# imperatormk/candle-birefnet

Hardware: AMD Instinct MI355X
Metric: images/sec @1024x1024 Swin-L (higher is better)
Workload: dtype f32 storage+accumulate; GEMM operands as two fp16 planes of the power-of-two-scaled operand (22-bit mantissa), 3 fp16 MFMAs/product (fp32-equivalent inside the fp16 range: |GEMM input| < 8190); 1 GPU; BASELINE configs[1]: Swin-L 1024x1024 batch=1 fp32 on 1xMI355X (single-image latency); batch_per_gpu=1, global_batch=1, size=1024, deform_mode=reference_cpu, compute=f32_half2, streams_per_gpu=1, branch_streams_per_gpu=5, inputs=resident in HBM (torch cuda tensors), weights: synthetic seed 42

## Files before the change

candle_birefnet_amd/csrc/kernels/window_attention.hip:

```cpp
#include "../brn_kernels.h"
#include "split_planes.h"
#include <cstdlib>
#include <type_traits>

namespace brn {

typedef float f32x4 __attribute__((ext_vector_type(4)));

constexpr int WS = 12;
constexpr int NTOK = 144;
constexpr int HD = 32;
constexpr int KV_LD = 36;
constexpr int ATT_THREADS = 192;

template <int IOB>
__device__ __forceinline__ f32x4 att_load4(const float* base, long off) {
    if constexpr (IOB != 0) {
        using E = std::conditional_t<IOB == 2, _Float16, __bf16>;
        typedef E ex4_ld __attribute__((ext_vector_type(4)));
        const ex4_ld h = *reinterpret_cast<const ex4_ld*>(reinterpret_cast<const E*>(base) + off);
        return f32x4{(float)h[0], (float)h[1], (float)h[2], (float)h[3]};
    } else return *reinterpret_cast<const f32x4*>(base + off);
}
template <int IOB>
__device__ __forceinline__ f32x4 att_bias4(const float* bias) {
    f32x4 v = *reinterpret_cast<const f32x4*>(bias);
    if constexpr (IOB != 0) {
        using E = std::conditional_t<IOB == 2, _Float16, __bf16>;
#pragma unroll
        for (int e = 0; e < 4; ++e) v[e] = (float)(E)v[e];
    }
    return v;
}
template <int WSZ, int NWV = 3, int IOB = 0>
__global__ void __launch_bounds__(NWV * 64) window_attention_f32_kernel(const WindowAttnParams pa, const WindowAttnParams pb, const int nblk0) {
    constexpr int WS = WSZ, NTOK = WSZ * WSZ, NT16 = (NTOK + 15) / 16, NPADTOK = NT16 * 16;
    constexpr int NTHR = NWV * 64;
    const bool second = (int)blockIdx.x >= nblk0;
    const WindowAttnParams& p = second ? pb : pa;
    __shared__ __attribute__((aligned(16))) float Ks[NPADTOK * KV_LD];
    __shared__ __attribute__((aligned(16))) float Vs[NPADTOK * KV_LD];
    __shared__ int src_s[NPADTOK];
    __shared__ int rid_s[NPADTOK];
    __shared__ float tab_s[(2 * WS - 1) * (2 * WS - 1)];

    const int tid = threadIdx.x, lane = tid & 63, wave = tid >> 6;
    const int head = blockIdx.y;
    const int nWw = p.Wp / WS, nW = (p.Hp / WS) * nWw;
    const int bw = second ? (int)blockIdx.x - nblk0 : (int)blockIdx.x;
    const int b = bw / nW, w = bw - b * nW;
    const int wr = w / nWw, wc = w - wr * nWw;
    const int C = p.C, C3 = 3 * C;

    if (tid < NTOK) {
        const int ti = tid / WS, tj = tid - ti * WS;
        const int ph = wr * WS + ti, pw = wc * WS + tj;
        int sh = ph + p.shift, sw = pw + p.shift;
        if (sh >= p.Hp) sh -= p.Hp;
        if (sw >= p.Wp) sw -= p.Wp;
        src_s[tid] = (sh < p.H && sw < p.W) ? (b * p.H + sh) * p.W + sw : -1;
        const int fh = ph < p.Hp - WS ? 0 : (ph < p.Hp - p.shift ? 1 : 2);
        const int fw = pw < p.Wp - WS ? 0 : (pw < p.Wp - p.shift ? 1 : 2);
        rid_s[tid] = fh * 3 + fw;
    } else if (tid < NPADTOK) { src_s[tid] = -1; rid_s[tid] = 0; }
    constexpr int TABN = (2 * WS - 1) * (2 * WS - 1);
    constexpr bool REV = WS == 12;
    constexpr float LOG2E = 1.4426950408889634f;
    for (int i = tid; i < TABN; i += NTHR) tab_s[i] = REV ? LOG2E * p.rel_table[head * TABN + (TABN - 1 - i)] : p.rel_table[head * TABN + i];
    const bool has_mask = p.shift > 0 && (wr == p.Hp / WS - 1 || wc == nWw - 1);
    __syncthreads();

    for (int idx = tid; idx < NPADTOK * 8; idx += NTHR) {
        const int t = idx >> 3, c4 = (idx & 7) * 4;
        const int src = src_s[t];
        f32x4 kv, vv;
        if (src >= 0) { kv = att_load4<IOB>(p.qkv, (long)src * C3 + C + head * HD + c4); vv = att_load4<IOB>(p.qkv, (long)src * C3 + 2 * C + head * HD + c4); }
        else { kv = att_bias4<IOB>(p.qkv_bias + C + head * HD + c4); vv = att_bias4<IOB>(p.qkv_bias + 2 * C + head * HD + c4); }
        if (t >= NTOK) { kv = f32x4{0.f, 0.f, 0.f, 0.f}; vv = kv; }
        *reinterpret_cast<f32x4*>(Ks + t * KV_LD + c4) = kv;
        *reinterpret_cast<f32x4*>(Vs + t * KV_LD + c4) = vv;
    }
    __syncthreads();

    const int li = lane & 15, g = lane >> 4;

    auto load_q = [&](int qt, f32x4& q0, f32x4& q1) {
        const int qs = src_s[qt * 16 + li];
        if (qs >= 0) { q0 = att_load4<IOB>(p.qkv, (long)qs * C3 + head * HD + g * 8); q1 = att_load4<IOB>(p.qkv, (long)qs * C3 + head * HD + g * 8 + 4); }
        else { q0 = att_bias4<IOB>(p.qkv_bias + head * HD + g * 8); q1 = att_bias4<IOB>(p.qkv_bias + head * HD + g * 8 + 4); }
    };
    f32x4 qn0 = {0.f, 0.f, 0.f, 0.f}, qn1 = qn0;
    if (wave < NT16) load_q(wave, qn0, qn1);
    for (int qt = wave; qt < NT16; qt += NWV) {
        const int qtok = qt * 16 + li;
        const int qsrc = src_s[qtok];
        const int qrid = rid_s[qtok];
        const int qt_ = qtok < NTOK ? qtok : NTOK - 1;
        const int qbase = (qt_ / WS + WS - 1) * (2 * WS - 1) + (qt_ % WS) + WS - 1;
        float qf[8];
#pragma unroll
        for (int e = 0; e < 4; ++e) { qf[e] = qn0[e] * p.scale; qf[4 + e] = qn1[e] * p.scale; }
        if (qt + NWV < NT16) load_q(qt + NWV, qn0, qn1);
        f32x4 st[NT16];
#pragma unroll
        for (int kt = 0; kt < NT16; ++kt) {
            const float* kp = Ks + (kt * 16 + li) * KV_LD + g * 8;
            const f32x4 k0 = *reinterpret_cast<const f32x4*>(kp);
            const f32x4 k1 = *reinterpret_cast<const f32x4*>(kp + 4);
            f32x4 acc = {0.f, 0.f, 0.f, 0.f};
#pragma unroll
            for (int e = 0; e < 4; ++e) acc = __builtin_amdgcn_mfma_f32_16x16x4f32(k0[e], qf[e], acc, 0, 0, 0);
#pragma unroll
            for (int e = 0; e < 4; ++e) acc = __builtin_amdgcn_mfma_f32_16x16x4f32(k1[e], qf[4 + e], acc, 0, 0, 0);
            st[kt] = acc;
            if (kt % 3 == 2) __builtin_amdgcn_sched_barrier(0);
        }
        float mx = -3.0e38f;
        if constexpr (REV) {
            const int qrev = (TABN - 1) - qbase;
#pragma unroll
            for (int kt = 0; kt < NT16; ++kt) {
                const int key0 = kt * 16 + g * 4;
                const float* tb = tab_s + qrev + key0 + (WS - 1) * (key0 / WS);
#pragma unroll
                for (int r = 0; r < 4; ++r) st[kt][r] = fmaf(st[kt][r], LOG2E, tb[r]);
            }
            if (has_mask) {
#pragma unroll
                for (int kt = 0; kt < NT16; ++kt) {
#pragma unroll
                    for (int r = 0; r < 4; ++r) st[kt][r] += (rid_s[kt * 16 + g * 4 + r] != qrid) ? -100.0f * LOG2E : 0.0f;
                }
            }
#pragma unroll
            for (int kt = 0; kt < NT16; ++kt) mx = fmaxf(fmaxf(mx, fmaxf(st[kt][0], st[kt][1])), fmaxf(st[kt][2], st[kt][3]));
        } else {
#pragma unroll
            for (int kt = 0; kt < NT16; ++kt) {
#pragma unroll
                for (int r = 0; r < 4; ++r) {
                    const int key = kt * 16 + g * 4 + r;
                    const int kk = key < NTOK ? key : 0;
                    float s = st[kt][r] + tab_s[max(0, qbase - kk - (WS - 1) * (kk / WS))];
                    if (p.shift > 0) s += (rid_s[key] != qrid) ? -100.0f : 0.0f;
                    if (NTOK % 16 != 0 && key >= NTOK) s = -3.0e38f;
                    st[kt][r] = s;
                    mx = fmaxf(mx, s);
                }
            }
        }
        mx = fmaxf(mx, __shfl_xor(mx, 16));
        mx = fmaxf(mx, __shfl_xor(mx, 32));
        float sum = 0.f;
#pragma unroll
        for (int kt = 0; kt < NT16; ++kt) {
#pragma unroll
            for (int r = 0; r < 4; ++r) {
                const float e = REV ? __builtin_amdgcn_exp2f(st[kt][r] - mx) : __expf(st[kt][r] - mx);
                st[kt][r] = e;
                sum += e;
            }
        }
        sum += __shfl_xor(sum, 16);
        sum += __shfl_xor(sum, 32);
        f32x4 o0 = {0.f, 0.f, 0.f, 0.f}, o1 = {0.f, 0.f, 0.f, 0.f};
#pragma unroll
        for (int kt = 0; kt < NT16; ++kt) {
#pragma unroll
            for (int r = 0; r < 4; ++r) {
                const float* vp = Vs + (kt * 16 + g * 4 + r) * KV_LD + li;
                o0 = __builtin_amdgcn_mfma_f32_16x16x4f32(vp[0], st[kt][r], o0, 0, 0, 0);
                o1 = __builtin_amdgcn_mfma_f32_16x16x4f32(vp[16], st[kt][r], o1, 0, 0, 0);
            }
            if (kt % 2 == 1) __builtin_amdgcn_sched_barrier(0);
        }
        if (qsrc >= 0 && qtok < NTOK) {
            const float inv = 1.0f / sum;
            if (p.out_planes == 3) {
                float* orow = p.out + (long)qsrc * (C + C / 2);
                store_planes<3>(orow, head * HD + g * 4, o0 * inv);
                store_planes<3>(orow, head * HD + 16 + g * 4, o1 * inv);
            } else if (p.out_planes == 2) {
                float* orow = p.out + (long)qsrc * C;
                store_planes_h(orow, head * HD + g * 4, o0 * inv, p.out_h2);
                store_planes_h(orow, head * HD + 16 + g * 4, o1 * inv, p.out_h2);
            } else if constexpr (IOB != 0) {
                using E = std::conditional_t<IOB == 2, _Float16, __bf16>;
                typedef E ex4_st __attribute__((ext_vector_type(4)));
                E* op = reinterpret_cast<E*>(p.out) + (long)qsrc * C + head * HD + g * 4;
                ex4_st h0, h1;
#pragma unroll
                for (int e = 0; e < 4; ++e) { h0[e] = (E)(o0[e] * inv); h1[e] = (E)(o1[e] * inv); }
                *reinterpret_cast<ex4_st*>(op) = h0;
                *reinterpret_cast<ex4_st*>(op + 16) = h1;
            } else {
                float* op = p.out + (long)qsrc * C + head * HD + g * 4;
                *reinterpret_cast<f32x4*>(op) = o0 * inv;
                *reinterpret_cast<f32x4*>(op + 16) = o1 * inv;
            }
        }
    }
}

typedef __bf16 bf16x8 __attribute__((ext_vector_type(8)));
typedef __bf16 bf16x4 __attribute__((ext_vector_type(4)));
typedef __bf16 bf16x2 __attribute__((ext_vector_type(2)));
constexpr int VT_LD = 148;

__device__ __forceinline__ int kswz(int key) { return (0x78 >> (2 * ((key >> 2) & 3))) & 3; }

constexpr float ATT_H_QKV = 8.0f, ATT_H_P = 2048.0f;
template <int NP, bool H = false>
__global__ void __launch_bounds__(ATT_THREADS) window_attention_split_kernel(const WindowAttnParams pa, const WindowAttnParams pb, const int nblk0) {
    static_assert(!H || NP == 2, "fp16 planes come in pairs");
    const bool second = (int)blockIdx.x >= nblk0;
    const WindowAttnParams& p = second ? pb : pa;
    __shared__ __attribute__((aligned(16))) __bf16 Kp[NP * NTOK * HD];
    __shared__ __attribute__((aligned(16))) __bf16 Vt[NP * HD * VT_LD];
    __shared__ float tab_s[(2 * WS - 1) * (2 * WS - 1)];
    __shared__ int src_s[NTOK];
    __shared__ unsigned char rid_s[NTOK];

    const int tid = threadIdx.x, lane = tid & 63, wave = tid >> 6;
    const int head = blockIdx.y;
    const int nWw = p.Wp / WS, nW = (p.Hp / WS) * nWw;
    const int bw = second ? (int)blockIdx.x - nblk0 : (int)blockIdx.x;
    const int b = bw / nW, w = bw - b * nW;
    const int wr = w / nWw, wc = w - wr * nWw;
    const int C = p.C, C3 = 3 * C;

    if (tid < NTOK) {
        const int ti = tid / WS, tj = tid - ti * WS;
        const int ph = wr * WS + ti, pw = wc * WS + tj;
        int sh = ph + p.shift, sw = pw + p.shift;
        if (sh >= p.Hp) sh -= p.Hp;
        if (sw >= p.Wp) sw -= p.Wp;
        src_s[tid] = (sh < p.H && sw < p.W) ? (b * p.H + sh) * p.W + sw : -1;
        const int fh = ph < p.Hp - WS ? 0 : (ph < p.Hp - p.shift ? 1 : 2);
        const int fw = pw < p.Wp - WS ? 0 : (pw < p.Wp - p.shift ? 1 : 2);
        rid_s[tid] = (unsigned char)(fh * 3 + fw);
    }
    for (int i = tid; i < (2 * WS - 1) * (2 * WS - 1); i += ATT_THREADS) tab_s[i] = p.rel_table[head * ((2 * WS - 1) * (2 * WS - 1)) + i];
    __syncthreads();

    for (int idx = tid; idx < (NTOK / 2) * 8; idx += ATT_THREADS) {
        const int tp = idx >> 3, c4 = (idx & 7) * 4;
        f32x4 kv[2], vv[2];
#pragma unroll
        for (int u = 0; u < 2; ++u) {
            const int t = tp * 2 + u, src = src_s[t];
            const float* kp = src >= 0 ? p.qkv + (long)src * C3 + C + head * HD + c4 : p.qkv_bias + C + head * HD + c4;
            kv[u] = *reinterpret_cast<const f32x4*>(kp);
            vv[u] = *reinterpret_cast<const f32x4*>(kp + C);
        }
        if constexpr (H) {
#pragma unroll
            for (int u = 0; u < 2; ++u) {
                const int t = tp * 2 + u;
                bf16x4 sp[2];
                split4h<false>(kv[u], 0xffffffffu, ATT_H_QKV, sp);
#pragma unroll
                for (int pl = 0; pl < 2; ++pl)
                    *reinterpret_cast<bf16x4*>(Kp + (pl * NTOK + t) * HD + (((c4 >> 3) ^ kswz(t)) << 3) + (c4 & 4)) = sp[pl];
            }
#pragma unroll
            for (int e = 0; e < 4; ++e) {
                unsigned hi, lo;
                split_pair_h(vv[0][e], vv[1][e], ATT_H_QKV, hi, lo);
                *reinterpret_cast<unsigned*>(Vt + (c4 + e) * VT_LD + tp * 2) = hi;
                *reinterpret_cast<unsigned*>(Vt + (HD + c4 + e) * VT_LD + tp * 2) = lo;
            }
        } else {
#pragma unroll
        for (int u = 0; u < 2; ++u) {
            const int t = tp * 2 + u;
            f32x4 r = kv[u];
#pragma unroll
            for (int pl = 0; pl < NP; ++pl) {
                bf16x4 h;
#pragma unroll
                for (int e = 0; e < 4; ++e) h[e] = (__bf16)r[e];
                *reinterpret_cast<bf16x4*>(Kp + (pl * NTOK + t) * HD + (((c4 >> 3) ^ kswz(t)) << 3) + (c4 & 4)) = h;
                if (pl + 1 < NP) {
#pragma unroll
                    for (int e = 0; e < 4; ++e) r[e] -= (float)h[e];
                }
            }
        }
        f32x4 r0 = vv[0], r1 = vv[1];
#pragma unroll
        for (int pl = 0; pl < NP; ++pl) {
#pragma unroll
            for (int e = 0; e < 4; ++e) {
                bf16x2 h;
                h[0] = (__bf16)r0[e]; h[1] = (__bf16)r1[e];
                *reinterpret_cast<bf16x2*>(Vt + (pl * HD + c4 + e) * VT_LD + tp * 2) = h;
                if (pl + 1 < NP) { r0[e] -= (float)h[0]; r1[e] -= (float)h[1]; }
            }
        }
        }
    }
    __syncthreads();

    const int li = lane & 15, g = lane >> 4;
    for (int qt = wave; qt < 9; qt += 3) {
        const int qtok = qt * 16 + li;
        const int qsrc = src_s[qtok];
        const int qrid = rid_s[qtok];
        const int qbase = (qtok / WS + WS - 1) * (2 * WS - 1) + (qtok % WS) + WS - 1;
        bf16x8 qf[NP];
        {
            const float* qp = qsrc >= 0 ? p.qkv + (long)qsrc * C3 + head * HD + g * 8 : p.qkv_bias + head * HD + g * 8;
            const f32x4 q0 = *reinterpret_cast<const f32x4*>(qp);
            const f32x4 q1 = *reinterpret_cast<const f32x4*>(qp + 4);
            float r[8];
#pragma unroll
            for (int e = 0; e < 4; ++e) { r[e] = q0[e] * p.scale; r[4 + e] = q1[e] * p.scale; }
            if constexpr (H) {
                typedef unsigned u32x4_q __attribute__((ext_vector_type(4)));
                u32x4_q hi, lo;
#pragma unroll
                for (int e = 0; e < 4; ++e) { unsigned a, b2; split_pair_h(r[2 * e], r[2 * e + 1], ATT_H_QKV, a, b2); hi[e] = a; lo[e] = b2; }
                qf[0] = __builtin_bit_cast(bf16x8, hi);
                qf[1] = __builtin_bit_cast(bf16x8, lo);
            } else {
#pragma unroll
            for (int pl = 0; pl < NP; ++pl) {
#pragma unroll
                for (int e = 0; e < 8; ++e) {
                    const __bf16 h = (__bf16)r[e];
                    qf[pl][e] = h;
                    r[e] -= (float)h;
                }
            }
            }
        }
        f32x4 st[9];
#pragma unroll
        for (int kt = 0; kt < 9; ++kt) {
            const int key = kt * 16 + li;
            bf16x8 kf[NP];
#pragma unroll
            for (int pl = 0; pl < NP; ++pl)
                kf[pl] = *reinterpret_cast<const bf16x8*>(Kp + (pl * NTOK + key) * HD + ((g ^ kswz(key)) << 3));
            f32x4 acc = {0.f, 0.f, 0.f, 0.f};
            if constexpr (H) {
                acc = __builtin_amdgcn_mfma_f32_16x16x32_f16(__builtin_bit_cast(f16x8, kf[1]), __builtin_bit_cast(f16x8, qf[0]), acc, 0, 0, 0);
                acc = __builtin_amdgcn_mfma_f32_16x16x32_f16(__builtin_bit_cast(f16x8, kf[0]), __builtin_bit_cast(f16x8, qf[1]), acc, 0, 0, 0);
                acc = __builtin_amdgcn_mfma_f32_16x16x32_f16(__builtin_bit_cast(f16x8, kf[0]), __builtin_bit_cast(f16x8, qf[0]), acc, 0, 0, 0);
            } else {
            if (NP == 2) {
                acc = __builtin_amdgcn_mfma_f32_16x16x32_bf16(kf[1], qf[0], acc, 0, 0, 0);
                acc = __builtin_amdgcn_mfma_f32_16x16x32_bf16(kf[0], qf[1], acc, 0, 0, 0);
            }
            acc = __builtin_amdgcn_mfma_f32_16x16x32_bf16(kf[0], qf[0], acc, 0, 0, 0);
            }
            st[kt] = acc;
            if (kt % 3 == 2) __builtin_amdgcn_sched_barrier(0);
        }
        float mx = -3.0e38f;
#pragma unroll
        for (int kt = 0; kt < 9; ++kt) {
#pragma unroll
            for (int r = 0; r < 4; ++r) {
                const int key = kt * 16 + g * 4 + r;
                float sv = H ? fmaf(st[kt][r], 1.0f / (ATT_H_QKV * ATT_H_QKV), tab_s[qbase - key - 11 * (key / WS)]) : st[kt][r] + tab_s[qbase - key - 11 * (key / WS)];
                if (p.shift > 0) sv += ((int)rid_s[key] != qrid) ? -100.0f : 0.0f;
                st[kt][r] = sv;
                mx = fmaxf(mx, sv);
            }
        }
        mx = fmaxf(mx, __shfl_xor(mx, 16));
        mx = fmaxf(mx, __shfl_xor(mx, 32));
        float sum = 0.f;
#pragma unroll
        for (int kt = 0; kt < 9; ++kt) {
#pragma unroll
            for (int r = 0; r < 4; ++r) {
                const float e = __expf(st[kt][r] - mx);
                st[kt][r] = e;
                sum += e;
            }
        }
        sum += __shfl_xor(sum, 16);
        sum += __shfl_xor(sum, 32);
        f32x4 o0 = {0.f, 0.f, 0.f, 0.f}, o1 = {0.f, 0.f, 0.f, 0.f};
#pragma unroll
        for (int t = 0; t < 5; ++t) {
            bf16x8 pf[NP];
            {
                float r[8];
#pragma unroll
                for (int e = 0; e < 4; ++e) { r[e] = st[2 * t][e]; r[4 + e] = (2 * t + 1 < 9) ? st[(2 * t + 1 < 9) ? 2 * t + 1 : 0][e] : 0.f; }
                if constexpr (H) {
                    typedef unsigned u32x4_p __attribute__((ext_vector_type(4)));
                    u32x4_p hi, lo;
#pragma unroll
                    for (int e = 0; e < 4; ++e) { unsigned a, b2; split_pair_h(r[2 * e], r[2 * e + 1], ATT_H_P, a, b2); hi[e] = a; lo[e] = b2; }
                    pf[0] = __builtin_bit_cast(bf16x8, hi);
                    pf[1] = __builtin_bit_cast(bf16x8, lo);
                } else {
#pragma unroll
                for (int pl = 0; pl < NP; ++pl) {
#pragma unroll
                    for (int e = 0; e < 8; ++e) {
                        const __bf16 h = (__bf16)r[e];
                        pf[pl][e] = h;
                        r[e] -= (float)h;
                    }
                }
                }
            }
#pragma unroll
            for (int dt = 0; dt < 2; ++dt) {
                bf16x8 vf[NP];
#pragma unroll
                for (int pl = 0; pl < NP; ++pl) {
                    const __bf16* vrow = Vt + (pl * HD + dt * 16 + li) * VT_LD + g * 4;
                    const bf16x4 lo = *reinterpret_cast<const bf16x4*>(vrow + (2 * t) * 16);
                    bf16x4 hi = {(__bf16)0.f, (__bf16)0.f, (__bf16)0.f, (__bf16)0.f};
                    if (2 * t + 1 < 9) hi = *reinterpret_cast<const bf16x4*>(vrow + (2 * t + 1) * 16);
#pragma unroll
                    for (int e = 0; e < 4; ++e) { vf[pl][e] = lo[e]; vf[pl][4 + e] = hi[e]; }
                }
                f32x4 o = dt == 0 ? o0 : o1;
                if constexpr (H) {
                    o = __builtin_amdgcn_mfma_f32_16x16x32_f16(__builtin_bit_cast(f16x8, vf[1]), __builtin_bit_cast(f16x8, pf[0]), o, 0, 0, 0);
                    o = __builtin_amdgcn_mfma_f32_16x16x32_f16(__builtin_bit_cast(f16x8, vf[0]), __builtin_bit_cast(f16x8, pf[1]), o, 0, 0, 0);
                    o = __builtin_amdgcn_mfma_f32_16x16x32_f16(__builtin_bit_cast(f16x8, vf[0]), __builtin_bit_cast(f16x8, pf[0]), o, 0, 0, 0);
                } else {
                if (NP == 2) {
                    o = __builtin_amdgcn_mfma_f32_16x16x32_bf16(vf[1], pf[0], o, 0, 0, 0);
                    o = __builtin_amdgcn_mfma_f32_16x16x32_bf16(vf[0], pf[1], o, 0, 0, 0);
                }
                o = __builtin_amdgcn_mfma_f32_16x16x32_bf16(vf[0], pf[0], o, 0, 0, 0);
                }
                if (dt == 0) o0 = o; else o1 = o;
            }
            __builtin_amdgcn_sched_barrier(0);
        }
        if (qsrc >= 0) {
            const float inv = (H ? 1.0f / (ATT_H_P * ATT_H_QKV) : 1.0f) / sum;
            if (H && p.out_planes == 2) {
                float* orow = p.out + (long)qsrc * C;
                store_planes_h(orow, head * HD + g * 4, o0 * inv, p.out_h2);
                store_planes_h(orow, head * HD + 16 + g * 4, o1 * inv, p.out_h2);
            } else if (p.out_planes == 2) {
                float* orow = p.out + (long)qsrc * C;
                store_planes<2>(orow, head * HD + g * 4, o0 * inv);
                store_planes<2>(orow, head * HD + 16 + g * 4, o1 * inv);
            } else {
                float* op = p.out + (long)qsrc * C + head * HD + g * 4;
                *reinterpret_cast<f32x4*>(op) = o0 * inv;
                *reinterpret_cast<f32x4*>(op + 16) = o1 * inv;
            }
        }
    }
}

__device__ __forceinline__ float max3f(float a, float b, float c) {
    float r;
    asm("v_max3_f32 %0, %1, %2, %3" : "=v"(r) : "v"(a), "v"(b), "v"(c));
    return r;
}
template <typename E>
__device__ __forceinline__ auto bias8_s16(const float* bp) {
    typedef E ex8_b __attribute__((ext_vector_type(8)));
    ex8_b r;
#pragma unroll
    for (int e = 0; e < 8; ++e) r[e] = (E)bp[e];
    return r;
}

template <int ATT_BF16_HPW, bool F16 = false>
__global__ void __launch_bounds__(ATT_BF16_HPW * ATT_THREADS) __attribute__((amdgpu_waves_per_eu(5, 8))) window_attention_bf16_kernel(const WindowAttnParams pa, const WindowAttnParams pb, const int nblk0) {
    using E = std::conditional_t<F16, _Float16, __bf16>;
    typedef E ex8 __attribute__((ext_vector_type(8)));
    typedef E ex4 __attribute__((ext_vector_type(4)));
    typedef E ex2 __attribute__((ext_vector_type(2)));
    auto mfma = [](const ex8 a, const ex8 b, const f32x4 c) -> f32x4 {
        if constexpr (F16) return __builtin_amdgcn_mfma_f32_16x16x32_f16(a, b, c, 0, 0, 0);
        else return __builtin_amdgcn_mfma_f32_16x16x32_bf16(a, b, c, 0, 0, 0);
    };
    const bool second = (int)blockIdx.x >= nblk0;
    const WindowAttnParams& p = second ? pb : pa;
    constexpr int TABN = (2 * WS - 1) * (2 * WS - 1);
    constexpr float LOG2E = 1.4426950408889634f;
    __shared__ __attribute__((aligned(16))) E Kp_[ATT_BF16_HPW][NTOK * HD];
    __shared__ __attribute__((aligned(16))) E Vt_[ATT_BF16_HPW][HD * VT_LD];
    __shared__ float rev_[ATT_BF16_HPW][TABN + 3];
    __shared__ __attribute__((aligned(4))) unsigned char rid_s[NTOK];

    const int tid = threadIdx.x, lane = tid & 63, wave = tid >> 6;
    const int hp = wave / 3, wv = wave - 3 * hp;
    const int head = blockIdx.y * ATT_BF16_HPW + hp;
    const int nWh = p.Hp / WS, nWw = p.Wp / WS, nW = nWh * nWw;
    const int bw = second ? (int)blockIdx.x - nblk0 : (int)blockIdx.x;
    const int b = bw / nW, w = bw - b * nW;
    const int wr = w / nWw, wc = w - wr * nWw;
    const int C = p.C, C3 = 3 * C;
    const E* qkv = reinterpret_cast<const E*>(p.qkv);
    const int li = lane & 15, g = lane >> 4;
    const bool has_mask = p.shift > 0 && (wr == nWh - 1 || wc == nWw - 1);
    E* Kp = Kp_[hp];
    E* Vt = Vt_[hp];
    const float* rev_s = rev_[hp];

    auto tok_src = [&](int t) {
        const int ti = t / WS, tj = t - ti * WS;
        int sh = wr * WS + ti + p.shift, sw = wc * WS + tj + p.shift;
        if (sh >= p.Hp) sh -= p.Hp;
        if (sw >= p.Wp) sw -= p.Wp;
        return (sh < p.H && sw < p.W) ? (b * p.H + sh) * p.W + sw : -1;
    };
    constexpr int NTHR = ATT_BF16_HPW * ATT_THREADS;
    constexpr int NITEM = (NTOK / 2) * 4 * ATT_BF16_HPW;
    constexpr int NTAB = ATT_BF16_HPW * TABN;
    static_assert(2 * NTHR >= NITEM && 3 * NTHR >= NTAB, "two staging items and three table words per thread cover a head group");
    ex8 qf[3];
    int qsrc_[3];
#pragma unroll
    for (int u = 0; u < 3; ++u) {
        const int qs = tok_src((wv + 3 * u) * 16 + li);
        qsrc_[u] = qs;
        qf[u] = *reinterpret_cast<const ex8*>(qkv + (long)max(qs, 0) * C3 + head * HD + g * 8);
    }
    float tbw[3];
#pragma unroll
    for (int j = 0; j < 3; ++j) {
        const int i = min(tid + j * NTHR, NTAB - 1), hh = i / TABN, jj = i - hh * TABN;
        tbw[j] = p.rel_table[(blockIdx.y * ATT_BF16_HPW + hh) * TABN + (TABN - 1 - jj)];
    }
    ex8 kv[2][2], vv[2][2];
    int ssrc[2][2];
#pragma unroll
    for (int it = 0; it < 2; ++it) {
        const int idx = min(tid + it * NTHR, NITEM - 1);
        const int c8 = (idx & 3) * 8, hh = (idx >> 2) & (ATT_BF16_HPW - 1), tp = idx / (4 * ATT_BF16_HPW);
        const int hd = (blockIdx.y * ATT_BF16_HPW + hh) * HD;
#pragma unroll
        for (int u = 0; u < 2; ++u) {
            const int src = tok_src(tp * 2 + u);
            ssrc[it][u] = src;
            const E* kp = qkv + (long)max(src, 0) * C3 + C + hd + c8;
            kv[it][u] = *reinterpret_cast<const ex8*>(kp);
            vv[it][u] = *reinterpret_cast<const ex8*>(kp + C);
        }
    }
    if (tid < NTOK) {
        const int ti = tid / WS, tj = tid - ti * WS;
        const int ph = wr * WS + ti, pw = wc * WS + tj;
        const int fh = ph < p.Hp - WS ? 0 : (ph < p.Hp - p.shift ? 1 : 2);
        const int fw = pw < p.Wp - WS ? 0 : (pw < p.Wp - p.shift ? 1 : 2);
        rid_s[tid] = (unsigned char)(fh * 3 + fw);
    }
#pragma unroll
    for (int j = 0; j < 3; ++j) {
        const int i = tid + j * NTHR;
        if (i < NTAB) { const int hh = i / TABN; rev_[hh][i - hh * TABN] = LOG2E * tbw[j]; }
    }
#pragma unroll
    for (int u = 0; u < 3; ++u)
        if (qsrc_[u] < 0) qf[u] = bias8_s16<E>(p.qkv_bias + head * HD + g * 8);
#pragma unroll
    for (int it = 0; it < 2; ++it) {
        const int idx = tid + it * NTHR;
        if (idx < NITEM) {
            const int c8 = (idx & 3) * 8, hh = (idx >> 2) & (ATT_BF16_HPW - 1), tp = idx / (4 * ATT_BF16_HPW);
            const int hd = (blockIdx.y * ATT_BF16_HPW + hh) * HD;
#pragma unroll
            for (int u = 0; u < 2; ++u) {
                if (ssrc[it][u] < 0) {
                    kv[it][u] = bias8_s16<E>(p.qkv_bias + C + hd + c8);
                    vv[it][u] = bias8_s16<E>(p.qkv_bias + 2 * C + hd + c8);
                }
            }
#pragma unroll
            for (int u = 0; u < 2; ++u) {
                const int t = tp * 2 + u;
                *reinterpret_cast<ex8*>(Kp_[hh] + t * HD + (((c8 >> 3) ^ kswz(t)) << 3)) = kv[it][u];
            }
#pragma unroll
            for (int e = 0; e < 8; ++e) {
                ex2 h;
                h[0] = vv[it][0][e]; h[1] = vv[it][1][e];
                *reinterpret_cast<ex2*>(Vt_[hh] + (c8 + e) * VT_LD + tp * 2) = h;
            }
        }
    }
    __syncthreads();

    const float scale2 = p.scale * LOG2E;
    ex8 ones8;
#pragma unroll
    for (int e = 0; e < 8; ++e) ones8[e] = (E)1.0f;
    typedef __attribute__((address_space(3))) const float lds_cfloat;
    unsigned koffb[9];
#pragma unroll
    for (int kt = 0; kt < 9; ++kt) { const int key0 = kt * 16 + g * 4; koffb[kt] = (unsigned)(key0 + 11 * (key0 / WS)) * 4u; }
#pragma unroll
    for (int u = 0; u < 3; ++u) {
        const int qt = wv + 3 * u;
        const int qtok = qt * 16 + li;
        const int qsrc = qsrc_[u];
        const unsigned qrid4 = 0x01010101u * (unsigned)rid_s[qtok];
        const int qrev = (TABN - 1) - ((qtok / WS + WS - 1) * (2 * WS - 1) + (qtok % WS) + WS - 1);
        f32x4 st[9];
#pragma unroll
        for (int kt = 0; kt < 9; ++kt) {
            const int key = kt * 16 + li;
            const ex8 kf = *reinterpret_cast<const ex8*>(Kp + key * HD + ((g ^ kswz(key)) << 3));
            f32x4 acc = {0.f, 0.f, 0.f, 0.f};
            st[kt] = mfma(kf, qf[u], acc);
            if (kt % 3 == 2) __builtin_amdgcn_sched_barrier(0);
        }
        float mx = -3.0e38f;
        unsigned tbq = (unsigned)(unsigned long)(lds_cfloat*)(rev_s + qrev);
        asm volatile("" : "+v"(tbq));
#pragma unroll
        for (int kt = 0; kt < 9; ++kt) {
            lds_cfloat* tb = (lds_cfloat*)(unsigned long)(tbq + koffb[kt]);
#pragma unroll
            for (int r = 0; r < 4; ++r) st[kt][r] = fmaf(st[kt][r], scale2, tb[r]);
        }
        if (has_mask) {
#pragma unroll
            for (int kt = 0; kt < 9; ++kt) {
                const unsigned xr = *reinterpret_cast<const unsigned*>(rid_s + kt * 16 + g * 4) ^ qrid4;
                const unsigned x = ((xr + 0x7f7f7f7fu) >> 7) & 0x01010101u;
#pragma unroll
                for (int r = 0; r < 4; ++r) st[kt][r] = fmaf((float)((x >> (8 * r)) & 0xffu), -100.0f * LOG2E, st[kt][r]);
            }
        }
#pragma unroll
        for (int kt = 0; kt < 9; ++kt) mx = max3f(max3f(mx, st[kt][0], st[kt][1]), st[kt][2], st[kt][3]);
        mx = fmaxf(mx, __shfl_xor(mx, 16));
        mx = fmaxf(mx, __shfl_xor(mx, 32));
#pragma unroll
        for (int kt = 0; kt < 9; ++kt) {
#pragma unroll
            for (int r = 0; r < 4; ++r) st[kt][r] = __builtin_amdgcn_exp2f(st[kt][r] - mx);
        }
        f32x4 o0 = {0.f, 0.f, 0.f, 0.f}, o1 = {0.f, 0.f, 0.f, 0.f}, osum = {0.f, 0.f, 0.f, 0.f};
#pragma unroll
        for (int t = 0; t < 5; ++t) {
            ex8 pf;
#pragma unroll
            for (int e = 0; e < 4; ++e) {
                pf[e] = (E)st[2 * t][e];
                pf[4 + e] = (2 * t + 1 < 9) ? (E)st[(2 * t + 1 < 9) ? 2 * t + 1 : 0][e] : (E)0.f;
            }
#pragma unroll
            for (int dt = 0; dt < 2; ++dt) {
                const E* vrow = Vt + (dt * 16 + li) * VT_LD + g * 4;
                const ex4 lo = *reinterpret_cast<const ex4*>(vrow + (2 * t) * 16);
                ex4 hi = {(E)0.f, (E)0.f, (E)0.f, (E)0.f};
                if (2 * t + 1 < 9) hi = *reinterpret_cast<const ex4*>(vrow + (2 * t + 1) * 16);
                ex8 vf;
#pragma unroll
                for (int e = 0; e < 4; ++e) { vf[e] = lo[e]; vf[4 + e] = hi[e]; }
                if (dt == 0) o0 = mfma(vf, pf, o0);
                else o1 = mfma(vf, pf, o1);
            }
            osum = mfma(ones8, pf, osum);
            __builtin_amdgcn_sched_barrier(0);
        }
        if (qsrc >= 0) {
            const float inv = __builtin_amdgcn_rcpf(osum[0]);
            E* op = reinterpret_cast<E*>(p.out) + (long)qsrc * C + head * HD + g * 4;
            ex4 h0, h1;
#pragma unroll
            for (int e = 0; e < 4; ++e) { h0[e] = (E)(o0[e] * inv); h1[e] = (E)(o1[e] * inv); }
            *reinterpret_cast<ex4*>(op) = h0;
            *reinterpret_cast<ex4*>(op + 16) = h1;
        }
    }
}

static hipError_t check_attention(const WindowAttnParams& p) {
    const int ws = p.ws ? p.ws : WS;
    if (!(ws == 12 || ws == 7)) return hipErrorInvalidValue;
    if (p.C != p.heads * HD || p.Hp % ws || p.Wp % ws || p.Hp < p.H || p.Wp < p.W) return hipErrorInvalidValue;
    if (!(p.shift == 0 || p.shift == ws / 2)) return hipErrorInvalidValue;
    if (ws != WS && (p.planes || p.out_planes)) return hipErrorInvalidValue;
    return hipSuccess;
}
hipError_t launch_window_attention2(const WindowAttnParams& p, const WindowAttnParams* p2, hipStream_t s) {
    if (check_attention(p) != hipSuccess) return hipErrorInvalidValue;
    const int ws = p.ws ? p.ws : WS;
    const int n0 = p.B * (p.Hp / ws) * (p.Wp / ws);
    int n1 = 0;
    if (p2) {
        if ((p2->ws ? p2->ws : WS) != ws) return hipErrorInvalidValue;
        if (check_attention(*p2) != hipSuccess || p2->C != p.C || p2->heads != p.heads || p2->planes != p.planes || p2->out_planes != p.out_planes || p2->io_bf16 != p.io_bf16) return hipErrorInvalidValue;
        n1 = p2->B * (p2->Hp / ws) * (p2->Wp / ws);
    }
    if (p.out_planes && !((p.out_planes == 2 && p.planes == 2 && (p.out_h2 > 0.f) == (p.h2 != 0)) || (p.out_planes == 3 && p.planes == 0) || (p.out_planes == 2 && p.planes == 0 && p.out_h2 > 0.f && !p.io_bf16)))
        return hipErrorInvalidValue;
    if (p.h2 && (p.planes != 2 || p.io_bf16)) return hipErrorInvalidValue;
    if (p2 && (p2->out_h2 != p.out_h2 || p2->h2 != p.h2)) return hipErrorInvalidValue;
    const WindowAttnParams& q = p2 ? *p2 : p;
    dim3 grid(n0 + n1, p.heads), block(ATT_THREADS);
    if (p.io_bf16 && ws == 7) {
        if (p.out_planes || (p.C & 3)) return hipErrorInvalidValue;
        if (p.io_bf16 == 2) hipLaunchKernelGGL((window_attention_f32_kernel<7, 3, 2>), grid, block, 0, s, p, q, n0);
        else hipLaunchKernelGGL((window_attention_f32_kernel<7, 3, 1>), grid, block, 0, s, p, q, n0);
    } else if (p.io_bf16) {
        if (p.out_planes || (p.C & 7)) return hipErrorInvalidValue;
        static const bool two_heads = !(getenv("BRN_ATT_HPW") && atoi(getenv("BRN_ATT_HPW")) == 1);
        if (p.io_bf16 == 2) {
            if (two_heads && !(p.heads & 1)) hipLaunchKernelGGL((window_attention_bf16_kernel<2, true>), dim3(n0 + n1, p.heads / 2), dim3(2 * ATT_THREADS), 0, s, p, q, n0);
            else hipLaunchKernelGGL((window_attention_bf16_kernel<1, true>), grid, block, 0, s, p, q, n0);
        } else if (two_heads && !(p.heads & 1)) hipLaunchKernelGGL(window_attention_bf16_kernel<2>, dim3(n0 + n1, p.heads / 2), dim3(2 * ATT_THREADS), 0, s, p, q, n0);
        else hipLaunchKernelGGL(window_attention_bf16_kernel<1>, grid, block, 0, s, p, q, n0);
    } else if (p.planes == 2 && p.h2) hipLaunchKernelGGL((window_attention_split_kernel<2, true>), grid, block, 0, s, p, q, n0);
    else if (p.planes == 2) hipLaunchKernelGGL(window_attention_split_kernel<2>, grid, block, 0, s, p, q, n0);
#ifdef BRN_DIAG_BUILD
    else if (p.planes == 1) hipLaunchKernelGGL(window_attention_split_kernel<1>, grid, block, 0, s, p, q, n0);
#else
    else if (p.planes == 1) return hipErrorInvalidValue;
#endif
    else if (ws == 7) hipLaunchKernelGGL(window_attention_f32_kernel<7>, grid, block, 0, s, p, q, n0);
    else {
        static const int f32_waves = getenv("BRN_ATT_F32_WAVES") ? atoi(getenv("BRN_ATT_F32_WAVES")) : 9;
        if (f32_waves == 9) hipLaunchKernelGGL((window_attention_f32_kernel<12, 9>), grid, dim3(9 * 64), 0, s, p, q, n0);
        else hipLaunchKernelGGL((window_attention_f32_kernel<12, 3>), grid, block, 0, s, p, q, n0);
    }
    return hipGetLastError();
}
hipError_t launch_window_attention(const WindowAttnParams& p, hipStream_t s) { return launch_window_attention2(p, nullptr, s); }

}
```

Measured before the change: 93.56 images/s.

## Prefetch window attention K/V/Q loads into registers before staging barrier

The split window-attention kernel now issues all K/V global loads, relative-position table words and the first Q tile's loads into registers up front, computing token sources inline instead of through a shared src_s array and an extra barrier. It also prefetches the next Q tile during the current one, adds a waves_per_eu(3,3) occupancy hint, and skips the shift mask for interior windows that cannot contain mixed regions. The aim is to hide global-load latency and remove a barrier plus redundant mask work. In exchange, register pressure rises substantially, which the occupancy hint caps and which may cause spilling.

Result: faster. 94.51 images/s (median of 6 runs) (+1.0%).

```diff
diff --git a/candle_birefnet_amd/csrc/kernels/window_attention.hip b/candle_birefnet_amd/csrc/kernels/window_attention.hip
--- a/candle_birefnet_amd/csrc/kernels/window_attention.hip
+++ b/candle_birefnet_amd/csrc/kernels/window_attention.hip
@@ -211,47 +211,84 @@
 
 constexpr float ATT_H_QKV = 8.0f, ATT_H_P = 2048.0f;
 template <int NP, bool H = false>
-__global__ void __launch_bounds__(ATT_THREADS) window_attention_split_kernel(const WindowAttnParams pa, const WindowAttnParams pb, const int nblk0) {
+__global__ void __launch_bounds__(ATT_THREADS) __attribute__((amdgpu_waves_per_eu(3, 3))) window_attention_split_kernel(const WindowAttnParams pa, const WindowAttnParams pb, const int nblk0) {
     static_assert(!H || NP == 2, "fp16 planes come in pairs");
     const bool second = (int)blockIdx.x >= nblk0;
     const WindowAttnParams& p = second ? pb : pa;
     __shared__ __attribute__((aligned(16))) __bf16 Kp[NP * NTOK * HD];
     __shared__ __attribute__((aligned(16))) __bf16 Vt[NP * HD * VT_LD];
-    __shared__ float tab_s[(2 * WS - 1) * (2 * WS - 1)];
-    __shared__ int src_s[NTOK];
+    constexpr int TABN = (2 * WS - 1) * (2 * WS - 1);
+    __shared__ float tab_s[TABN];
     __shared__ unsigned char rid_s[NTOK];
+    __shared__ __attribute__((aligned(16))) float qb_s[HD];
 
     const int tid = threadIdx.x, lane = tid & 63, wave = tid >> 6;
+    const int li = lane & 15, g = lane >> 4;
     const int head = blockIdx.y;
     const int nWw = p.Wp / WS, nW = (p.Hp / WS) * nWw;
     const int bw = second ? (int)blockIdx.x - nblk0 : (int)blockIdx.x;
     const int b = bw / nW, w = bw - b * nW;
     const int wr = w / nWw, wc = w - wr * nWw;
     const int C = p.C, C3 = 3 * C;
+    const bool has_mask = p.shift > 0 && (wr == p.Hp / WS - 1 || wc == nWw - 1);
+
+    auto tok_src = [&](int t) {
+        const int ti = t / WS, tj = t - ti * WS;
+        int sh = wr * WS + ti + p.shift, sw = wc * WS + tj + p.shift;
+        if (sh >= p.Hp) sh -= p.Hp;
+        if (sw >= p.Wp) sw -= p.Wp;
+        return (sh < p.H && sw < p.W) ? (b * p.H + sh) * p.W + sw : -1;
+    };
+    static_assert((NTOK / 2) * 8 == 3 * ATT_THREADS && ATT_THREADS % 8 == 0 && 3 * ATT_THREADS >= TABN, "three staging items and three table words per thread");
+    const int c4 = (tid & 7) * 4;
+    const float* kbp = p.qkv_bias + C + head * HD + c4;
+    const f32x4 kbias = *reinterpret_cast<const f32x4*>(kbp);
+    const f32x4 vbias = *reinterpret_cast<const f32x4*>(kbp + C);
+    f32x4 kvr[3][2], vvr[3][2];
+    int ssrc[3][2];
+#pragma unroll
+    for (int it = 0; it < 3; ++it) {
+#pragma unroll
+        for (int u = 0; u < 2; ++u) {
+            const int src = tok_src(((tid >> 3) + it * (ATT_THREADS / 8)) * 2 + u);
+            ssrc[it][u] = src;
+            const float* kp = p.qkv + (long)max(src, 0) * C3 + C + head * HD + c4;
+            kvr[it][u] = *reinterpret_cast<const f32x4*>(kp);
+            vvr[it][u] = *reinterpret_cast<const f32x4*>(kp + C);
+        }
+    }
+    float tbw[3];
+#pragma unroll
+    for (int j = 0; j < 3; ++j) tbw[j] = p.rel_table[head * TABN + min(tid + j * ATT_THREADS, TABN - 1)];
+    const float* qbp = p.qkv_bias + head * HD + g * 8;
+    const f32x4 qbias0 = *reinterpret_cast<const f32x4*>(qbp);
+    const f32x4 qbias1 = *reinterpret_cast<const f32x4*>(qbp + 4);
+    int qsrc_n;
+    f32x4 qn0, qn1;
+    auto load_q = [&](int qtok) {
+        qsrc_n = tok_src(qtok);
+        const float* qp = p.qkv + (long)max(qsrc_n, 0) * C3 + head * HD + g * 8;
+        qn0 = *reinterpret_cast<const f32x4*>(qp);
+        qn1 = *reinterpret_cast<const f32x4*>(qp + 4);
+    };
+    load_q(wave * 16 + li);
 
     if (tid < NTOK) {
         const int ti = tid / WS, tj = tid - ti * WS;
         const int ph = wr * WS + ti, pw = wc * WS + tj;
-        int sh = ph + p.shift, sw = pw + p.shift;
-        if (sh >= p.Hp) sh -= p.Hp;
-        if (sw >= p.Wp) sw -= p.Wp;
-        src_s[tid] = (sh < p.H && sw < p.W) ? (b * p.H + sh) * p.W + sw : -1;
         const int fh = ph < p.Hp - WS ? 0 : (ph < p.Hp - p.shift ? 1 : 2);
         const int fw = pw < p.Wp - WS ? 0 : (pw < p.Wp - p.shift ? 1 : 2);
         rid_s[tid] = (unsigned char)(fh * 3 + fw);
     }
-    for (int i = tid; i < (2 * WS - 1) * (2 * WS - 1); i += ATT_THREADS) tab_s[i] = p.rel_table[head * ((2 * WS - 1) * (2 * WS - 1)) + i];
-    __syncthreads();
-
-    for (int idx = tid; idx < (NTOK / 2) * 8; idx += ATT_THREADS) {
-        const int tp = idx >> 3, c4 = (idx & 7) * 4;
+
+#pragma unroll
+    for (int it = 0; it < 3; ++it) {
+        const int tp = (tid >> 3) + it * (ATT_THREADS / 8);
         f32x4 kv[2], vv[2];
 #pragma unroll
         for (int u = 0; u < 2; ++u) {
-            const int t = tp * 2 + u, src = src_s[t];
-            const float* kp = src >= 0 ? p.qkv + (long)src * C3 + C + head * HD + c4 : p.qkv_bias + C + head * HD + c4;
-            kv[u] = *reinterpret_cast<const f32x4*>(kp);
-            vv[u] = *reinterpret_cast<const f32x4*>(kp + C);
+            kv[u] = ssrc[it][u] < 0 ? kbias : kvr[it][u];
+            vv[u] = ssrc[it][u] < 0 ? vbias : vvr[it][u];
         }
         if constexpr (H) {
 #pragma unroll
@@ -300,22 +337,28 @@
         }
         }
     }
+#pragma unroll
+    for (int j = 0; j < 3; ++j)
+        if (tid + j * ATT_THREADS < TABN) tab_s[tid + j * ATT_THREADS] = tbw[j];
+    if (tid < 64 && li == 0) {
+        *reinterpret_cast<f32x4*>(qb_s + g * 8) = qbias0;
+        *reinterpret_cast<f32x4*>(qb_s + g * 8 + 4) = qbias1;
+    }
     __syncthreads();
 
-    const int li = lane & 15, g = lane >> 4;
     for (int qt = wave; qt < 9; qt += 3) {
         const int qtok = qt * 16 + li;
-        const int qsrc = src_s[qtok];
+        const int qsrc = qsrc_n;
         const int qrid = rid_s[qtok];
         const int qbase = (qtok / WS + WS - 1) * (2 * WS - 1) + (qtok % WS) + WS - 1;
         bf16x8 qf[NP];
         {
-            const float* qp = qsrc >= 0 ? p.qkv + (long)qsrc * C3 + head * HD + g * 8 : p.qkv_bias + head * HD + g * 8;
-            const f32x4 q0 = *reinterpret_cast<const f32x4*>(qp);
-            const f32x4 q1 = *reinterpret_cast<const f32x4*>(qp + 4);
+            const f32x4 q0 = qsrc < 0 ? *reinterpret_cast<const f32x4*>(qb_s + g * 8) : qn0;
+            const f32x4 q1 = qsrc < 0 ? *reinterpret_cast<const f32x4*>(qb_s + g * 8 + 4) : qn1;
             float r[8];
 #pragma unroll
             for (int e = 0; e < 4; ++e) { r[e] = q0[e] * p.scale; r[4 + e] = q1[e] * p.scale; }
+            if (qt + 3 < 9) load_q(qtok + 48);
             if constexpr (H) {
                 typedef unsigned u32x4_q __attribute__((ext_vector_type(4)));
                 u32x4_q hi, lo;
@@ -365,7 +408,7 @@
             for (int r = 0; r < 4; ++r) {
                 const int key = kt * 16 + g * 4 + r;
                 float sv = H ? fmaf(st[kt][r], 1.0f / (ATT_H_QKV * ATT_H_QKV), tab_s[qbase - key - 11 * (key / WS)]) : st[kt][r] + tab_s[qbase - key - 11 * (key / WS)];
-                if (p.shift > 0) sv += ((int)rid_s[key] != qrid) ? -100.0f : 0.0f;
+                if (has_mask) sv += ((int)rid_s[key] != qrid) ? -100.0f : 0.0f;
                 st[kt][r] = sv;
                 mx = fmaxf(mx, sv);
             }
```
